# zeyadmohamedabdo/Visual-Question-Answering-VQA-system

Hardware: AMD Instinct MI355X
Metric: image-question pairs/sec (train step) (higher is better)
Workload: dtype bf16

## Files before the change

### visual-question-answering-vqa-system_amd/csrc/cnn_ops.hip

```cpp
#include "common.h"
#include "stem_route.h"

__global__ void bn_reduce_partials_kernel(const float* __restrict__ part, double* __restrict__ acc, int tiles, int C) {
  const int c = blockIdx.x * 64 + (threadIdx.x & 63), tl = threadIdx.x >> 6;
  __shared__ double sh[2][4][64];
  double s = 0.0, q = 0.0;
  if (c < C) {
    const int step = gridDim.y * 4;
    int t = blockIdx.y * 4 + tl;
    for (; t + 7 * step < tiles; t += 8 * step) {
      float a[8], b[8];
#pragma unroll
      for (int u = 0; u < 8; ++u) { a[u] = part[((size_t)(t + u * step) * 2) * C + c]; b[u] = part[((size_t)(t + u * step) * 2 + 1) * C + c]; }
#pragma unroll
      for (int u = 0; u < 8; ++u) { s += (double)a[u]; q += (double)b[u]; }
    }
    for (; t < tiles; t += step) {
      s += (double)part[((size_t)t * 2) * C + c];
      q += (double)part[((size_t)t * 2 + 1) * C + c];
    }
  }
  sh[0][tl][threadIdx.x & 63] = s; sh[1][tl][threadIdx.x & 63] = q;
  __syncthreads();
  if (tl == 0 && c < C) {
// ... 314 lines not shown
    const int ch = c0 + j;
    a[j] = cf[ch]; b[j] = cf[C + ch]; c[j] = cf[2 * C + ch];
    if (DUAL) { a2[j] = cf[3 * C + ch]; b2[j] = cf[4 * C + ch]; c2[j] = cf[5 * C + ch]; }
    if (SELF) { ms[j] = coef[ch]; mh[j] = coef[C + ch]; }
  }
#pragma unroll 2
  for (size_t r = (size_t)blockIdx.x * lanes_r + myr; r < rows; r += (size_t)gridDim.x * lanes_r) {
    const size_t off = r * C + c0;
    Vec16<T> d = ldg16(dout + off), yy = ldg16(y + off), o, y2v, rr, r2;
    if (!SELF && outact) o = ldg16(outact + off);
    if (DUAL) y2v = ldg16(y2 + off);
#pragma unroll
    for (int j = 0; j < VEC; ++j) {
      float g = d.get(j);
      if (SELF) { if (!(yy.get(j) * ms[j] + mh[j] > 0.f)) g = 0.f; }
      else if (outact && !(o.get(j) > 0.f)) g = 0.f;
      rr.set(j, a[j] * g + b[j] * yy.get(j) + c[j]);
      if (DUAL) r2.set(j, a2[j] * g + b2[j] * y2v.get(j) + c2[j]);
    }
    stg16(dy + off, rr);
    if (DUAL) stg16(dy2 + off, r2);
  }
}

constexpr int SP_ROWS = 4, SP_PAIRS = 7;
template <typename T>
__global__ __launch_bounds__(256) void stem_pool_fwd_kernel(const T* __restrict__ y, const float* __restrict__ coef, T* __restrict__ out,
                                                            uint8_t* __restrict__ idx, int B, int H, int W, int C, int Ho, int Wo, int trows) {
  constexpr int VEC = Vec16<T>::N;
  const int cv = C / VEC, Wp = (Wo + 1) >> 1;
  const int tiles_x = (Wp + SP_PAIRS - 1) / SP_PAIRS, tiles_y = (Ho + trows - 1) / trows;
  const int per_row = SP_PAIRS * cv;
  const int ry = threadIdx.x / per_row, rem = threadIdx.x - ry * per_row;
  if (ry >= trows) return;
  const int pr = rem / cv, c0 = (rem - pr * cv) * VEC;
  int t = blockIdx.x;
  const int tx = t % tiles_x; t /= tiles_x; const int ty = t % tiles_y; const int b = t / tiles_y;
  const int oh = ty * trows + ry, owp = tx * SP_PAIRS + pr;
  if (oh >= Ho || owp >= Wp) return;
  float sc[VEC], sh[VEC];
#pragma unroll
  for (int j = 0; j < VEC; ++j) { sc[j] = coef[c0 + j]; sh[j] = coef[C + c0 + j]; }
  const int ow0 = owp * 2;
  const bool two = ow0 + 1 < Wo;
  float best[2][VEC]; int bi[2][VEC];
#pragma unroll
  for (int o = 0; o < 2; ++o)
#pragma unroll
    for (int j = 0; j < VEC; ++j) { best[o][j] = -INFINITY; bi[o][j] = 0; }
#pragma unroll
  for (int r = 0; r < 3; ++r) {
    const int ih = oh * 2 - 1 + r;
    if (ih < 0 || ih >= H) continue;
    const T* yr = y + (((size_t)b * H + ih) * W) * C + c0;
#pragma unroll
    for (int s5 = 0; s5 < 5; ++s5) {
      const int iw = ow0 * 2 - 1 + s5;
      if (iw < 0 || iw >= W) continue;
      const Vec16<T> yy = ldg16(yr + (size_t)iw * C);
      float a[VEC];
#pragma unroll
      for (int j = 0; j < VEC; ++j) { const float v = yy.get(j) * sc[j] + sh[j]; a[j] = v < 0.f ? 0.f : v; }
      if (s5 < 3) {
#pragma unroll
        for (int j = 0; j < VEC; ++j)
          if (a[j] > best[0][j] || a[j] != a[j]) { best[0][j] = a[j]; bi[0][j] = r * 3 + s5; }
      }
      if (s5 >= 2) {
#pragma unroll
        for (int j = 0; j < VEC; ++j)
          if (a[j] > best[1][j] || a[j] != a[j]) { best[1][j] = a[j]; bi[1][j] = r * 3 + s5 - 2; }
      }
    }
  }
#pragma unroll
  for (int o = 0; o < 2; ++o) {
    if (o == 1 && !two) break;
    const size_t e = ((((size_t)b * Ho + oh) * Wo + ow0 + o) * C + c0);
    Vec16<T> ov;
    uint32_t pk[VEC / 4];
#pragma unroll
    for (int q4 = 0; q4 < VEC / 4; ++q4) pk[q4] = 0u;
#pragma unroll
    for (int j = 0; j < VEC; ++j) { ov.set(j, best[o][j]); pk[j >> 2] |= (uint32_t)bi[o][j] << (8 * (j & 3)); }
    stg16(out + e, ov);
#pragma unroll
    for (int q4 = 0; q4 < VEC / 4; ++q4) reinterpret_cast<uint32_t*>(idx + e)[q4] = pk[q4];
  }
}

template <typename T>
__global__ __launch_bounds__(256) void stem_bwd_reduce_kernel(const T* __restrict__ dpool, const uint8_t* __restrict__ idx, const T* __restrict__ y,
                                                              const float* __restrict__ coef, float* __restrict__ slab,
                                                              int B, int H, int W, int C, int Ho, int Wo) {
  constexpr int VEC = Vec16<T>::N;
  const int cv = C / VEC, lanes_r = 256 / cv;
  const int myv = threadIdx.x % cv, myr = threadIdx.x / cv, c0 = myv * VEC;
  const size_t rows = (size_t)B * H * W;
  float sg[VEC], sx[VEC], g[VEC], sc[VEC], sh[VEC], mean[VEC], inv[VEC];
#pragma unroll
  for (int j = 0; j < VEC; ++j) { sg[j] = sx[j] = 0.f; sc[j] = coef[c0 + j]; sh[j] = coef[C + c0 + j]; mean[j] = coef[2 * C + c0 + j]; inv[j] = coef[3 * C + c0 + j]; }
  if (myr < lanes_r)
    for (size_t r = (size_t)blockIdx.x * lanes_r + myr; r < rows; r += (size_t)gridDim.x * lanes_r) {
      const int w = (int)(r % W); size_t q = r / W; const int h = (int)(q % H); const int b = (int)(q / H);
      Vec16<T> yy = ldg16(y + r * C + c0);
      stem_route<T>(dpool, idx, yy, sc, sh, b, h, w, c0, C, Ho, Wo, g);
#pragma unroll
      for (int j = 0; j < VEC; ++j) { sg[j] += g[j]; sx[j] += g[j] * (yy.get(j) - mean[j]) * inv[j]; }
    }
  extern __shared__ float shm[];
#pragma unroll
  for (int j = 0; j < VEC; ++j) { shm[(0 * 256 + threadIdx.x) * VEC + j] = sg[j]; shm[(1 * 256 + threadIdx.x) * VEC + j] = sx[j]; }
  __syncthreads();
  for (int o = threadIdx.x; o < 2 * C; o += 256) {
    const int k = o / C, c = o - k * C, v = c / VEC, j = c - v * VEC;
    float s = 0.f;
    for (int r = 0; r < lanes_r; ++r) s += shm[(k * 256 + r * cv + v) * VEC + j];
    slab[((size_t)blockIdx.x * 3 + k) * C + c] = s;
    if (k == 0) slab[((size_t)blockIdx.x * 3 + 2) * C + c] = 0.f;
  }
}

template <typename T>
__global__ void stem_bwd_apply_kernel(const T* __restrict__ dpool, const uint8_t* __restrict__ idx, const T* __restrict__ y,
                                      const float* __restrict__ coef, const float* __restrict__ bc, T* __restrict__ dy,
                                      int B, int H, int W, int C, int Ho, int Wo) {
  constexpr int VEC = Vec16<T>::N;
  const int cv = C / VEC;
  const size_t total = (size_t)B * H * W * cv;
  float g[VEC];
  for (size_t i = (size_t)blockIdx.x * blockDim.x + threadIdx.x; i < total; i += (size_t)gridDim.x * blockDim.x) {
    const int v = (int)(i % cv); size_t r = i / cv;
    const int w = (int)(r % W); size_t q = r / W; const int h = (int)(q % H); const int b = (int)(q / H);
    const int c0 = v * VEC;
    Vec16<T> yy = ldg16(y + i * VEC), o;
    float sc[VEC], sh[VEC];
#pragma unroll
    for (int j = 0; j < VEC; ++j) { sc[j] = coef[c0 + j]; sh[j] = coef[C + c0 + j]; }
    stem_route<T>(dpool, idx, yy, sc, sh, b, h, w, c0, C, Ho, Wo, g);
#pragma unroll
    for (int j = 0; j < VEC; ++j) o.set(j, bc[c0 + j] * g[j] + bc[C + c0 + j] * yy.get(j) + bc[2 * C + c0 + j]);
    stg16(dy + i * VEC, o);
  }
}

template <typename T>
__global__ __launch_bounds__(256) void se_pool_fc_kernel(const T* __restrict__ x, const float* __restrict__ w1, const float* __restrict__ w2,
                                                         float* __restrict__ pooled, float* __restrict__ hidden, float* __restrict__ scale,
                                                         int HW, int C, int Cr, const float* __restrict__ part, int chunks) {
  constexpr int VEC = Vec16<T>::N;
  extern __shared__ float sh[];
  const int b = blockIdx.x, cv = C / VEC, lanes_r = 256 / cv;
  const int myv = threadIdx.x % cv, myr = threadIdx.x / cv;
  float s[VEC];
#pragma unroll
  for (int j = 0; j < VEC; ++j) s[j] = 0.f;
  if (!part && myr < lanes_r) {
    const T* xb = x + (size_t)b * HW * C + myv * VEC;
    int p = myr;
    for (; p + 3 * lanes_r < HW; p += 4 * lanes_r) {
      Vec16<T> v0 = ldg16(xb + (size_t)p * C), v1 = ldg16(xb + (size_t)(p + lanes_r) * C);
      Vec16<T> v2 = ldg16(xb + (size_t)(p + 2 * lanes_r) * C), v3 = ldg16(xb + (size_t)(p + 3 * lanes_r) * C);
#pragma unroll
      for (int j = 0; j < VEC; ++j) s[j] += (v0.get(j) + v1.get(j)) + (v2.get(j) + v3.get(j));
    }
    for (; p < HW; p += lanes_r) {
      Vec16<T> v = ldg16(xb + (size_t)p * C);
// ... 861 lines not shown
```

### visual-question-answering-vqa-system_amd/csrc/common.h

```cpp
#pragma once
#include <hip/hip_runtime.h>
#include <stdint.h>

#include <stdlib.h>

#ifdef VQA_ABLATION
static inline int vqa_env_int(const char* name, int dflt) { const char* e = getenv(name); return e ? atoi(e) : dflt; }
#else
static inline int vqa_env_int(const char*, int dflt) { return dflt; }
#endif

#define VQA_OK 0
#define VQA_EARG 1000

typedef uint16_t bf16_t;
typedef __attribute__((ext_vector_type(4))) float f32x4;
typedef __attribute__((ext_vector_type(8))) __bf16 bf16x8;
typedef __attribute__((ext_vector_type(4))) short i16x4;
typedef __attribute__((ext_vector_type(4))) uint32_t u32x4;

__device__ __forceinline__ float bf2f(bf16_t v) { return __uint_as_float(((uint32_t)v) << 16); }
__device__ __forceinline__ bf16_t f2bf(float f) {
  __bf16 b = (__bf16)f;
  return __builtin_bit_cast(bf16_t, b);
}
template <typename T> __device__ __forceinline__ float to_f(T v);
template <> __device__ __forceinline__ float to_f<float>(float v) { return v; }
template <> __device__ __forceinline__ float to_f<bf16_t>(bf16_t v) { return bf2f(v); }
template <typename T> __device__ __forceinline__ T from_f(float v);
template <> __device__ __forceinline__ float from_f<float>(float v) { return v; }
template <> __device__ __forceinline__ bf16_t from_f<bf16_t>(float v) { return f2bf(v); }

template <typename T> struct Vec16;
template <> struct Vec16<float> {
  static constexpr int N = 4;
  u32x4 raw;
  __device__ __forceinline__ float get(int i) const { return __uint_as_float(raw[i]); }
  __device__ __forceinline__ void set(int i, float v) { raw[i] = __float_as_uint(v); }
};
template <> struct Vec16<bf16_t> {
  static constexpr int N = 8;
  u32x4 raw;
  __device__ __forceinline__ float get(int i) const {
    uint32_t w = raw[i >> 1];
    return __uint_as_float((i & 1) ? (w & 0xffff0000u) : (w << 16));
  }
  __device__ __forceinline__ void set(int i, float v) {
    uint32_t b = f2bf(v);
    uint32_t w = raw[i >> 1];
    raw[i >> 1] = (i & 1) ? ((w & 0x0000ffffu) | (b << 16)) : ((w & 0xffff0000u) | b);
  }
};
template <typename T> __device__ __forceinline__ Vec16<T> ldg16(const T* p) {
  Vec16<T> v; v.raw = *reinterpret_cast<const u32x4*>(p); return v;
}
template <typename T> __device__ __forceinline__ void stg16(T* p, const Vec16<T>& v) {
  *reinterpret_cast<u32x4*>(p) = v.raw;
}
template <typename T> __device__ __forceinline__ Vec16<T> zero16() {
  Vec16<T> v; v.raw = u32x4{0u, 0u, 0u, 0u}; return v;
}

__device__ __forceinline__ float wave_sum(float v) {
#pragma unroll
  for (int o = 32; o > 0; o >>= 1) v += __shfl_xor(v, o, 64);
  return v;
}
__device__ __forceinline__ float wave_max(float v) {
#pragma unroll
  for (int o = 32; o > 0; o >>= 1) v = fmaxf(v, __shfl_xor(v, o, 64));
  return v;
}

__device__ __forceinline__ uint32_t mix32(uint32_t x) {
  x ^= x >> 16; x *= 0x7feb352dU; x ^= x >> 15; x *= 0x846ca68bU; x ^= x >> 16; return x;
}
__device__ __forceinline__ uint32_t drop_key(uint64_t seed) { return mix32((uint32_t)seed) ^ (uint32_t)(seed >> 32) * 0x9E3779B9u; }
__device__ __forceinline__ bool drop_keep32(uint32_t key, uint32_t idx, float p) {
  const uint32_t h = mix32(idx ^ key);
  return (float)(h >> 8) * (1.0f / 16777216.0f) >= p;
}
__device__ __forceinline__ bool drop_keep(uint64_t seed, uint64_t idx, float p) {
  uint32_t h = mix32((uint32_t)idx ^ mix32((uint32_t)(idx >> 32) + (uint32_t)seed) ^ (uint32_t)(seed >> 32) * 0x9E3779B9u);
  return (float)(h >> 8) * (1.0f / 16777216.0f) >= p;
}

static inline __host__ __device__ int acc_replicas(int C) { const int r = 512 / (C > 0 ? C : 1); return r < 1 ? 1 : (r > 8 ? 8 : r); }
#define VQA_ACC_HI_SHIFT 4
#define VQA_ACC_LO_SHIFT 50
#define VQA_ACC_MAX_PARTS (1 << 17)
#define VQA_ACC_LIMIT_LOG2 (62 - VQA_ACC_HI_SHIFT - 17)
__device__ __forceinline__ void acc_add_fixed(unsigned long long* acc, size_t n, size_t idx, float v) {
  constexpr float lim = (float)(1ull << VQA_ACC_LIMIT_LOG2), hs = (float)(1 << VQA_ACC_HI_SHIFT), lscale = (float)(1ull << VQA_ACC_LO_SHIFT);
  if (fabsf(v) < lim) {
    const float hi = rintf(v * hs);
    const float lo = __builtin_fmaf(hi, -1.f / hs, v);
    atomicAdd(acc + idx, (unsigned long long)(long long)hi);
    if (lo != 0.f) atomicAdd(acc + n + 1 + idx, (unsigned long long)__float2ll_rn(lo * lscale));
  } else atomicAdd(acc + n, 1ull);
}
__device__ __forceinline__ double acc_read_fixed(const unsigned long long* acc, int R, int K, int C, int k, int c) {
  const size_t n = (size_t)R * K * C;
  long long h[8], l[8];
#pragma unroll
  for (int r = 0; r < 8; ++r) {
    const size_t i = ((size_t)r * K + k) * C + c;
    h[r] = r < R ? (long long)acc[i] : 0ll;
// ... 33 lines not shown
```

### visual-question-answering-vqa-system_amd/csrc/stem_conv.hip

```cpp
#include <cstdlib>
#include "common.h"
#include <type_traits>
#include "stem_route.h"

namespace {
constexpr int RB = 4;
constexpr int PR = 2 * RB + 5;
constexpr int KP = 192;
constexpr int LDW = KP + 8;
constexpr int LDCS = 64 + 8;
}

template <int PROWS, int XO, int CH>
__device__ __forceinline__ void stem_fill_patch(bf16_t* __restrict__ patch, int PW, __amdgpu_buffer_rsrc_t rsImg, int b, int ih_base,
                                                int H, int W, int tid) {
  static_assert(XO & 1, "odd column offset");
  const int W4 = W >> 2, nitems = 3 * PROWS * W4, nh = PW - W;
  const float inv_w4 = 1.0f / (float)W4, inv_nh = 1.0f / (float)nh;
  for (int i = tid; i < 3 * PROWS * nh; i += 256) {
    const int row = (int)(((float)i + 0.5f) * inv_nh), k = i - row * nh;
    patch[row * PW + (k < XO ? k : W + k)] = 0;
  }
  for (int base = tid; base < nitems; base += 256 * CH) {
    f32x4 v[CH]; int dst[CH];
#pragma unroll
    for (int i = 0; i < CH; ++i) {
      const int id = base + 256 * i;
      dst[i] = -1;
      v[i] = f32x4{0.f, 0.f, 0.f, 0.f};
      if (id < nitems) {
        const int row = (int)(((float)id + 0.5f) * inv_w4), j = id - row * W4;
        const int c = row / PROWS, pr = row - c * PROWS, ih = ih_base + pr;
        dst[i] = row * PW + 4 * j + XO;
        if (ih >= 0 && ih < H)
          v[i] = __builtin_bit_cast(f32x4, __builtin_amdgcn_raw_buffer_load_b128(rsImg, (((b * 3 + c) * H + ih) * W + 4 * j) * 4, 0, 0));
      }
    }
#pragma unroll
    for (int i = 0; i < CH; ++i) {
      if (dst[i] < 0) continue;
      bf16_t* d = patch + dst[i];
      d[0] = f2bf(v[i][0]);
      *reinterpret_cast<uint32_t*>(d + 1) = (uint32_t)f2bf(v[i][1]) | ((uint32_t)f2bf(v[i][2]) << 16);
      d[3] = f2bf(v[i][3]);
    }
  }
}

__global__ void stem_pack_kernel(const float* __restrict__ w, bf16_t* __restrict__ out) {
  const int i = blockIdx.x * blockDim.x + threadIdx.x;
  if (i >= 64 * KP) return;
  const int n = i / KP, k = i - n * KP, pair = k >> 3, s = k & 7;
  float v = 0.f;
  if (pair < 21 && s < 7) { const int c = pair / 7, r = pair - c * 7; v = w[((n * 7 + r) * 7 + s) * 3 + c]; }
  out[i] = f2bf(v);
}

__global__ __launch_bounds__(256) void stem_conv_kernel(const float* __restrict__ img, const bf16_t* __restrict__ wst, bf16_t* __restrict__ out,
                                                        float* __restrict__ stats, int H, int W, int Ho, int Wo) {
  extern __shared__ __attribute__((aligned(16))) char smem[];
  const int PW = 2 * Wo + 8;
  bf16_t* patch = reinterpret_cast<bf16_t*>(smem);
  bf16_t* Wl = patch + 3 * PR * PW;
  bf16_t* Cst = Wl;
  float* red = reinterpret_cast<float*>(Wl + 64 * LDW);
  const int tid = threadIdx.x, lane = tid & 63, wave = tid >> 6, g = lane >> 4, li = lane & 15;
  const int rblocks = Ho / RB;
  const int b = blockIdx.x / rblocks, oh0 = (blockIdx.x - b * rblocks) * RB;

  for (int v = tid; v < 64 * (KP / 8); v += 256) {
    const int n = v / (KP / 8), kv = v - n * (KP / 8);
    *reinterpret_cast<u32x4*>(&Wl[n * LDW + kv * 8]) = *reinterpret_cast<const u32x4*>(&wst[n * KP + kv * 8]);
  }
  const int ih_base = 2 * oh0 - 3;
  const __amdgpu_buffer_rsrc_t rsImg = __builtin_amdgcn_make_buffer_rsrc(const_cast<float*>(img), 0, (int)gridDim.x / rblocks * 3 * H * W * 4, 0x00020000);
  for (int x = tid; x < PW; x += 256) {
    const int iw = x - 3;
    const bool cok = iw >= 0 && iw < W;
    float vals[3 * PR];
#pragma unroll
    for (int row = 0; row < 3 * PR; ++row) {
      const int c = row / PR, pr = row - c * PR, ih = ih_base + pr;
// ... 122 lines not shown
  for (int kk = 0; kk < 6; ++kk)
#pragma unroll
    for (int nt = 0; nt < 4; ++nt)
      bfr[kk][nt] = *reinterpret_cast<const bf16x8*>(&Wl[(nt * 16 + li) * LDW + kk * 32 + g * 8]);
  float sc[4], sh[4];
#pragma unroll
  for (int nt = 0; nt < 4; ++nt) { sc[nt] = coef[nt * 16 + li]; sh[nt] = coef[64 + nt * 16 + li]; }
  __syncthreads();
  if (dbg & 4) { if (tid == 0) out[(size_t)blockIdx.x * 64] = f2bf(sc[0] + (float)bfr[0][0][0]); return; }

  bf16_t* mycs = Cst + wave * 8 * LDCS;
  for (int t = wave; t < ctiles; t += 4) {
    const int c0 = 14 * t - 1;
    auto row = [&](int i, float (&h)[4][2]) {
      f32x4 acc[4];
#pragma unroll
      for (int nt = 0; nt < 4; ++nt) acc[nt] = f32x4{0.f, 0.f, 0.f, 0.f};
      if (!(dbg & 1))
#pragma unroll
      for (int kk = 0; kk < 6; ++kk) {
        int pair = kk * 4 + g;
        pair = pair > 20 ? 20 : pair;
        const int c = pair / 7, r = pair - c * 7;
        const uint32_t* ap = reinterpret_cast<const uint32_t*>(&patch[(c * PRP + 2 * i + r) * PW + 28 * t + 2 * li]);
        u32x4 raw = {ap[0], ap[1], ap[2], ap[3]};
        const bf16x8 af = __builtin_bit_cast(bf16x8, raw);
#pragma unroll
        for (int nt = 0; nt < 4; ++nt) acc[nt] = __builtin_amdgcn_mfma_f32_16x16x32_bf16(af, bfr[kk][nt], acc[nt], 0, 0, 0);
      }
      if (dbg & 2) {
#pragma unroll
        for (int nt = 0; nt < 4; ++nt) { h[nt][0] = acc[nt][0] + acc[nt][1]; h[nt][1] = acc[nt][2] + acc[nt][3]; }
        return;
      }
#pragma unroll
      for (int nt = 0; nt < 4; ++nt) {
        float v[4];
#pragma unroll
        for (int r4 = 0; r4 < 4; ++r4) {
          const int col = c0 + 4 * g + r4;
          const float a = acc[nt][r4] * sc[nt] + sh[nt];
          v[r4] = ((unsigned)col < (unsigned)Wo) ? (a < 0.f ? 0.f : a) : 0.f;
        }
        const float nx = __shfl_down(v[0], 16, 64);
        h[nt][0] = pool_max(pool_max(v[0], v[1]), v[2]);
        h[nt][1] = pool_max(pool_max(v[2], v[3]), nx);
      }
    };
    float hp[4][2], h1[4][2], h2[4][2];
    if (ph0 > 0) row(0, hp);
    else {
#pragma unroll
      for (int nt = 0; nt < 4; ++nt) { hp[nt][0] = 0.f; hp[nt][1] = 0.f; }
    }
#pragma unroll 1
    for (int k = 0; k < PRB; ++k) {
      row(2 * k + 1, h1);
      row(2 * k + 2, h2);
#pragma unroll
      for (int nt = 0; nt < 4; ++nt)
#pragma unroll
        for (int q = 0; q < 2; ++q) {
          const float o = pool_max(pool_max(hp[nt][q], h1[nt][q]), h2[nt][q]);
          mycs[(2 * g + q) * LDCS + nt * 16 + li] = f2bf(o);
          hp[nt][q] = h2[nt][q];
        }
      asm volatile("s_waitcnt lgkmcnt(0)" ::: "memory");
      const int px = lane >> 3, cv = lane & 7, pw = 7 * t + px;
      if (px < 7 && pw < Wp)
        *reinterpret_cast<u32x4*>(&out[((((size_t)b * Hp + ph0 + k) * Wp + pw) * 64) + cv * 8]) = *reinterpret_cast<const u32x4*>(&mycs[px * LDCS + cv * 8]);
      asm volatile("s_waitcnt lgkmcnt(0)" ::: "memory");
    }
  }
}

namespace {
constexpr int RBW = 4;
constexpr int PRW = 2 * RBW + 5;
constexpr int LDA = KP + 8;
constexpr int LDD = 64 + 4;
}

template <bool FUSED>
__global__ __launch_bounds__(256) void stem_wgrad_kernel(const float* __restrict__ img, const bf16_t* __restrict__ dy, float* __restrict__ dw,
                                                         int B, int H, int W, int Ho, int Wo, const bf16_t* __restrict__ dpool,
                                                         const uint8_t* __restrict__ idx, const float* __restrict__ coef,
                                                         const float* __restrict__ bc, int Hp, int Wp, int nsplit, float* __restrict__ ws) {
  extern __shared__ __attribute__((aligned(16))) char smem[];
  const int PW = 2 * Wo + 8;
  const int Wh = Wo / nsplit;
  const int MP = (Wh + 31) / 32 * 32;
  bf16_t* patch = reinterpret_cast<bf16_t*>(smem);
  bf16_t* Acol = patch + 3 * PRW * PW;
  bf16_t* Dy = Acol + MP * LDA;
  const int tid = threadIdx.x, lane = tid & 63, wave = tid >> 6, g = lane >> 4, li = lane & 15;
  const int q = li >> 2, pp = li & 3;
  for (int i = tid; i < (MP - Wh) * LDA; i += 256) Acol[Wh * LDA + i] = 0;
  for (int i = tid; i < (MP - Wh) * LDD; i += 256) Dy[Wh * LDD + i] = 0;

  float f_sc[8], f_sh[8], f_a[8], f_b[8], f_c[8];
  if (FUSED) {
    const int c0f = (tid & 7) * 8;
#pragma unroll
    for (int j = 0; j < 8; ++j) {
      f_sc[j] = coef[c0f + j]; f_sh[j] = coef[64 + c0f + j];
      f_a[j] = bc[c0f + j]; f_b[j] = bc[64 + c0f + j]; f_c[j] = bc[128 + c0f + j];
    }
  }
  const __amdgpu_buffer_rsrc_t rsP = __builtin_amdgcn_make_buffer_rsrc(const_cast<bf16_t*>(FUSED ? dpool : dy), 0, FUSED ? B * Hp * Wp * 64 * 2 : 0, 0x00020000);
  const __amdgpu_buffer_rsrc_t rsI = __builtin_amdgcn_make_buffer_rsrc(const_cast<uint8_t*>(FUSED ? idx : reinterpret_cast<const uint8_t*>(dy)), 0, FUSED ? B * Hp * Wp * 64 : 0, 0x00020000);
  const __amdgpu_buffer_rsrc_t rsImg = __builtin_amdgcn_make_buffer_rsrc(const_cast<float*>(img), 0, B * 3 * H * W * 4, 0x00020000);
  const __amdgpu_buffer_rsrc_t rsDy = __builtin_amdgcn_make_buffer_rsrc(const_cast<bf16_t*>(dy), 0, B * Ho * Wo * 64 * 2, 0x00020000);
  f32x4 acc[4][3];
#pragma unroll
  for (int i = 0; i < 4; ++i)
#pragma unroll
    for (int j = 0; j < 3; ++j) acc[i][j] = f32x4{0.f, 0.f, 0.f, 0.f};

  const int rblocks = Ho / RBW, nblocks = B * rblocks;
  for (int blk = blockIdx.x; blk < nblocks; blk += gridDim.x) {
    const int b = blk / rblocks, oh0 = (blk - b * rblocks) * RBW;
    __syncthreads();
    const int ih_base = 2 * oh0 - 3;
    for (int x = tid; x < PW; x += 256) {
      const int iw = x - 3;
      const bool cok = iw >= 0 && iw < W;
      float vals[3 * PRW];
#pragma unroll
      for (int row = 0; row < 3 * PRW; ++row) {
        const int c = row / PRW, pr = row - c * PRW, ih = ih_base + pr;
        const bool ok = cok && ih >= 0 && ih < H;
        const int ihc = min(max(ih, 0), H - 1), iwc = min(max(iw, 0), W - 1);
        const float t = __builtin_bit_cast(float, __builtin_amdgcn_raw_buffer_load_b32(rsImg, (((b * 3 + c) * H + ihc) * W + iwc) * 4, 0, 0));
        vals[row] = ok ? t : 0.f;
      }
#pragma unroll
      for (int row = 0; row < 3 * PRW; ++row) patch[row * PW + x] = f2bf(vals[row]);
    }
    for (int unit = 0; unit < RBW * nsplit; ++unit) {
      const int orow = unit / nsplit, px0 = (unit - orow * nsplit) * Wh;
      __syncthreads();
      const int dyr_b = (((b * Ho + oh0 + orow) * Wo + px0) * 64) * 2;
      if constexpr (FUSED) {
        auto stage_row = [&](auto odd) {
          for (int v = tid; v < (Wh >> 1) * 8; v += 256) {
            const int pq = v >> 3, cv = v & 7;
            Vec16<bf16_t> yy[2];
            yy[0].raw = __builtin_bit_cast(u32x4, __builtin_amdgcn_raw_buffer_load_b128(rsDy, dyr_b + (2 * pq) * 128 + cv * 16, 0, 0));
            yy[1].raw = __builtin_bit_cast(u32x4, __builtin_amdgcn_raw_buffer_load_b128(rsDy, dyr_b + (2 * pq + 1) * 128 + cv * 16, 0, 0));
            float g8[2][8];
            stem_route_pair_buf<decltype(odd)::value>(rsP, rsI, yy, f_sc, f_sh, b, oh0 + orow, (px0 >> 1) + pq, cv * 8, Hp, Wp, g8);
#pragma unroll
            for (int q2 = 0; q2 < 2; ++q2) {
              Vec16<bf16_t> o;
#pragma unroll
              for (int j = 0; j < 8; ++j) o.set(j, f_a[j] * g8[q2][j] + f_b[j] * yy[q2].get(j) + f_c[j]);
              uint32_t* d = reinterpret_cast<uint32_t*>(&Dy[(2 * pq + q2) * LDD + cv * 8]);
              d[0] = o.raw[0]; d[1] = o.raw[1]; d[2] = o.raw[2]; d[3] = o.raw[3];
            }
          }
        };
        if ((oh0 + orow) & 1) stage_row(std::true_type{});
        else stage_row(std::false_type{});
      } else {
        for (int v = tid; v < Wh * 8; v += 256) {
          const int px = v >> 3, cv = v & 7;
          const u32x4 val = __builtin_bit_cast(u32x4, __builtin_amdgcn_raw_buffer_load_b128(rsDy, dyr_b + v * 16, 0, 0));
          uint32_t* d = reinterpret_cast<uint32_t*>(&Dy[px * LDD + cv * 8]);
          d[0] = val[0]; d[1] = val[1]; d[2] = val[2]; d[3] = val[3];
        }
      }
      if (tid < 240) {
        const int pair = tid % 24, c = pair / 7, r = pair - c * 7;
        const bf16_t* prow = patch + (c * PRW + 2 * orow + r) * PW + 2 * px0;
        for (int px = tid / 24; px < Wh; px += 10) {
          u32x4 val = {0u, 0u, 0u, 0u};
          if (pair < 21) {
            const uint32_t* ap = reinterpret_cast<const uint32_t*>(prow + 2 * px);
            val = u32x4{ap[0], ap[1], ap[2], ap[3] & 0x0000ffffu};
          }
          *reinterpret_cast<u32x4*>(&Acol[px * LDA + pair * 8]) = val;
        }
      }
      __syncthreads();
      typedef __attribute__((ext_vector_type(8))) short i16x8;
      for (int ks = 0; ks < MP / 32; ++ks) {
        const bf16_t* yb = Dy + (ks * 32 + 8 * g + q) * LDD + 4 * pp;
        const bf16_t* xb = Acol + (ks * 32 + 8 * g + q) * LDA + wave * 48 + 4 * pp;
        bf16x8 af[4], bfv[3];
#pragma unroll
        for (int i = 0; i < 4; ++i) {
          i16x4 lo = __builtin_amdgcn_ds_read_tr16_b64_v4i16((i16x4 __attribute__((address_space(3)))*)(yb + i * 16));
          i16x4 hi = __builtin_amdgcn_ds_read_tr16_b64_v4i16((i16x4 __attribute__((address_space(3)))*)(yb + 4 * LDD + i * 16));
          i16x8 t = {lo[0], lo[1], lo[2], lo[3], hi[0], hi[1], hi[2], hi[3]};
          af[i] = __builtin_bit_cast(bf16x8, t);
        }
#pragma unroll
        for (int j = 0; j < 3; ++j) {
          i16x4 lo = __builtin_amdgcn_ds_read_tr16_b64_v4i16((i16x4 __attribute__((address_space(3)))*)(xb + j * 16));
          i16x4 hi = __builtin_amdgcn_ds_read_tr16_b64_v4i16((i16x4 __attribute__((address_space(3)))*)(xb + 4 * LDA + j * 16));
          i16x8 t = {lo[0], lo[1], lo[2], lo[3], hi[0], hi[1], hi[2], hi[3]};
          bfv[j] = __builtin_bit_cast(bf16x8, t);
        }
#pragma unroll
        for (int i = 0; i < 4; ++i)
#pragma unroll
          for (int j = 0; j < 3; ++j)
            acc[i][j] = __builtin_amdgcn_mfma_f32_16x16x32_bf16(af[i], bfv[j], acc[i][j], 0, 0, 0);
      }
    }
  }
#pragma unroll
  for (int j = 0; j < 3; ++j) {
    const int k2 = wave * 48 + j * 16 + li, pair = k2 >> 3, s = k2 & 7;
    if (pair >= 21 || s >= 7) continue;
    const int c = pair / 7, r = pair - c * 7;
#pragma unroll
    for (int i = 0; i < 4; ++i)
#pragma unroll
      for (int rr = 0; rr < 4; ++rr) {
        const size_t o = (size_t)(i * 16 + g * 4 + rr) * 147 + (r * 7 + s) * 3 + c;
        if (ws) ws[(size_t)blockIdx.x * (64 * 147) + o] = acc[i][j][rr];
        else atomicAdd(dw + o, acc[i][j][rr]);
      }
  }
}

extern "C" int vqa_slab_reduce(const float* ws, float* dw, int nslabs, long long n, hipStream_t st);

static size_t stem_wgrad_shm(int Wo, int nsplit) {
  const int PW = 2 * Wo + 8, MP = (Wo / nsplit + 31) / 32 * 32;
  return (size_t)(3 * PRW * PW + MP * LDA + MP * LDD) * 2;
}
static int stem_nsplit(int Wo) {
  const int env = vqa_env_int("VQA_STEM_NSPLIT", 0);
  if (env > 0 && Wo % (8 * env) == 0) return env;
  const int floor_ = Wo > 64 ? 2 : 1;
  for (int n = floor_; n <= 16; ++n)
    if (Wo % (8 * n) == 0 && stem_wgrad_shm(Wo, n) <= (size_t)160 * 1024 / 3) return n;
  return floor_;
}
static int stem_wgrad_grid(int B, int Ho, int Wo, size_t* shm_out) {
  const size_t shm = stem_wgrad_shm(Wo, stem_nsplit(Wo));
  if (shm_out) *shm_out = shm;
  if (shm > 160 * 1024) return 0;
  const int nblocks = B * (Ho / RBW);
  const int cap = 256 * (int)((160 * 1024) / shm > 4 ? 4 : (160 * 1024) / shm);
  return nblocks < cap ? nblocks : cap;
}

extern "C" {

int vqa_stem_conv_blocks(int B, int H, int W) {
  const int Ho = (H + 6 - 7) / 2 + 1, Wo = (W + 6 - 7) / 2 + 1;
  if (Ho % RB || Wo % 16 || Wo > 256) return 0;
  return B * (Ho / RB);
}
int vqa_stem_pack(const float* w_krsc, void* wstem , hipStream_t st) {
  if (!w_krsc || !wstem) return VQA_EARG;
  hipLaunchKernelGGL(stem_pack_kernel, dim3((64 * KP + 255) / 256), dim3(256), 0, st, w_krsc, (bf16_t*)wstem);
  VQA_LAUNCH_CHECK(); return VQA_OK;
}
int vqa_stem_conv(const float* img, const void* wstem, void* out, float* stats, int B, int H, int W, hipStream_t st) {
  const int nb = vqa_stem_conv_blocks(B, H, W);
  if (!img || !wstem || !out || nb <= 0 || (size_t)B * 3 * H * W * 4 >= 0x7fffffffull) return VQA_EARG;
  const int Ho = (H + 6 - 7) / 2 + 1, Wo = (W + 6 - 7) / 2 + 1, PW = 2 * Wo + 8;
  const size_t shm = (size_t)(3 * PR * PW + 64 * LDW) * 2 + 4 * 64 * 2 * 4;
  static size_t attr = 0;
  if (shm > attr) { (void)hipFuncSetAttribute(reinterpret_cast<const void*>(&stem_conv_kernel), hipFuncAttributeMaxDynamicSharedMemorySize, (int)shm); attr = shm; }
  hipLaunchKernelGGL(stem_conv_kernel, dim3(nb), dim3(256), shm, st, img, (const bf16_t*)wstem, (bf16_t*)out, stats, H, W, Ho, Wo);
  VQA_LAUNCH_CHECK(); return VQA_OK;
}

static size_t stem_conv_pool_shm(int H, int W, int* ctiles_out, int* pw_out) {
  const int Ho = (H + 6 - 7) / 2 + 1, Wo = (W + 6 - 7) / 2 + 1, Hp = (Ho + 2 - 3) / 2 + 1, Wp = (Wo + 2 - 3) / 2 + 1;
  if (H < 7 || W < 7 || (Ho & 1) || (Wo & 1) || Hp % PRB) return 0;
  const int ctiles = (Wp + 6) / 7;
  const int PW = (2 * (14 * ctiles + 2) + 8 + 7) / 8 * 8;
  if (ctiles_out) *ctiles_out = ctiles;
  if (pw_out) *pw_out = PW;
  const size_t shm = (size_t)(3 * PRP * PW + 64 * LDW) * 2;
  return shm <= 160 * 1024 ? shm : 0;
}
int vqa_stem_conv_pool_ok(int B, int H, int W) {
  return B > 0 && stem_conv_pool_shm(H, W, nullptr, nullptr) > 0 && (size_t)B * 3 * H * W * 4 < 0x7fffffffull;
}
int vqa_stem_conv_pool(const float* img, const void* wstem, const float* coef, void* out, int B, int H, int W, hipStream_t st) {
  int ctiles = 0, PW = 0;
  const size_t shm = stem_conv_pool_shm(H, W, &ctiles, &PW);
  if (!img || !wstem || !coef || !out || !vqa_stem_conv_pool_ok(B, H, W)) return VQA_EARG;
  const int Ho = (H + 6 - 7) / 2 + 1, Wo = (W + 6 - 7) / 2 + 1, Hp = (Ho + 2 - 3) / 2 + 1, Wp = (Wo + 2 - 3) / 2 + 1;
  static size_t attr = 0;
  if (shm > attr) { (void)hipFuncSetAttribute(reinterpret_cast<const void*>(&stem_conv_pool_kernel), hipFuncAttributeMaxDynamicSharedMemorySize, (int)shm); attr = shm; }
  hipLaunchKernelGGL(stem_conv_pool_kernel, dim3(B * (Hp / PRB)), dim3(256), shm, st, img, (const bf16_t*)wstem, coef, (bf16_t*)out,
                     B, H, W, Ho, Wo, Hp, Wp, ctiles, PW, vqa_env_int("VQA_STEMCP_DBG", 0));
  VQA_LAUNCH_CHECK(); return VQA_OK;
}

int vqa_stem_wgrad_blocks(int B, int H, int W) {
  const int Ho = (H + 6 - 7) / 2 + 1, Wo = (W + 6 - 7) / 2 + 1;
  if (Ho % RBW || Wo % 16 || Wo > 256) return 0;
  return stem_wgrad_grid(B, Ho, Wo, nullptr);
}

int vqa_stem_wgrad(const float* img, const void* dy, float* dw, int B, int H, int W, float* ws, long long ws_floats, hipStream_t st) {
  const int Ho = (H + 6 - 7) / 2 + 1, Wo = (W + 6 - 7) / 2 + 1;
  if (!img || !dy || !dw || Ho % RBW || Wo % 16 || Wo > 256) return VQA_EARG;
  if ((size_t)B * Ho * Wo * 64 * 2 >= 0x7fffffffull || (size_t)B * 3 * H * W * 4 >= 0x7fffffffull) return VQA_EARG;
  const int nsplit = stem_nsplit(Wo);
  const int PW = 2 * Wo + 8, MP = (Wo / nsplit + 31) / 32 * 32;
  const size_t shm = (size_t)(3 * PRW * PW + MP * LDA + MP * LDD) * 2;
  if (shm > 160 * 1024) return VQA_EARG;
  static size_t attr = 0;
  if (shm > attr) { (void)hipFuncSetAttribute(reinterpret_cast<const void*>(&stem_wgrad_kernel<false>), hipFuncAttributeMaxDynamicSharedMemorySize, (int)shm); attr = shm; }
  int nblocks = B * (Ho / RBW);
  const int cap = 256 * (int)((160 * 1024) / shm > 4 ? 4 : (160 * 1024) / shm);
  int grid = nblocks < cap ? nblocks : cap;
  float* w = (ws && ws_floats >= (long long)grid * 64 * 147) ? ws : nullptr;
  hipLaunchKernelGGL(stem_wgrad_kernel<false>, dim3(grid), dim3(256), shm, st, img, (const bf16_t*)dy, dw, B, H, W, Ho, Wo,
                     (const bf16_t*)nullptr, (const uint8_t*)nullptr, (const float*)nullptr, (const float*)nullptr, 0, 0, nsplit, w);
  VQA_LAUNCH_CHECK();
  return w ? vqa_slab_reduce(w, dw, grid, 64 * 147, st) : VQA_OK;
}
int vqa_stem_wgrad_fused(const float* img, const void* y, const void* dpool, const uint8_t* idx, const float* coef, const float* bcoef,
                         float* dw, int B, int H, int W, float* ws, long long ws_floats, hipStream_t st) {
  const int Ho = (H + 6 - 7) / 2 + 1, Wo = (W + 6 - 7) / 2 + 1, Hp = (Ho + 2 - 3) / 2 + 1, Wp = (Wo + 2 - 3) / 2 + 1;
  if (!img || !y || !dpool || !idx || !coef || !bcoef || !dw || Ho % RBW || Wo % 16 || Wo > 256) return VQA_EARG;
  if ((size_t)B * Ho * Wo * 64 * 2 >= 0x7fffffffull || (size_t)B * 3 * H * W * 4 >= 0x7fffffffull) return VQA_EARG;
  const int nsplit = stem_nsplit(Wo);
  const int PW = 2 * Wo + 8, MP = (Wo / nsplit + 31) / 32 * 32;
  const size_t shm = (size_t)(3 * PRW * PW + MP * LDA + MP * LDD) * 2;
  if (shm > 160 * 1024) return VQA_EARG;
  static size_t attr = 0;
  if (shm > attr) { (void)hipFuncSetAttribute(reinterpret_cast<const void*>(&stem_wgrad_kernel<true>), hipFuncAttributeMaxDynamicSharedMemorySize, (int)shm); attr = shm; }
  int nblocks = B * (Ho / RBW);
  const int cap = 256 * (int)((160 * 1024) / shm > 4 ? 4 : (160 * 1024) / shm);
  int grid = nblocks < cap ? nblocks : cap;
  float* w = (ws && ws_floats >= (long long)grid * 64 * 147) ? ws : nullptr;
  hipLaunchKernelGGL(stem_wgrad_kernel<true>, dim3(grid), dim3(256), shm, st, img, (const bf16_t*)y, dw, B, H, W, Ho, Wo,
                     (const bf16_t*)dpool, idx, coef, bcoef, Hp, Wp, nsplit, w);
  VQA_LAUNCH_CHECK();
  return w ? vqa_slab_reduce(w, dw, grid, 64 * 147, st) : VQA_OK;
}

}
```

### visual-question-answering-vqa-system_amd/csrc/stem_route.h

```cpp
#pragma once
#include "common.h"

template <typename T>
__device__ __forceinline__ void stem_route(const T* __restrict__ dpool, const uint8_t* __restrict__ idx, const Vec16<T>& yy,
                                           const float* sc, const float* sh, int b, int h, int w, int c0, int C, int Ho, int Wo, float* g) {
  constexpr int VEC = Vec16<T>::N;
#pragma unroll
  for (int j = 0; j < VEC; ++j) g[j] = 0.f;
  const int oh_a = (h - 1) >> 1, oh_b = (h + 1) >> 1, ow_a = (w - 1) >> 1, ow_b = (w + 1) >> 1;
  Vec16<T> d[4]; uint64_t iw4[4]; bool ok[4]; int code[4];
#pragma unroll
  for (int k = 0; k < 4; ++k) {
    const int oh = (k >> 1) ? oh_b : oh_a, ow = (k & 1) ? ow_b : ow_a;
    const int r = h - (oh * 2 - 1), s = w - (ow * 2 - 1);
    ok[k] = oh >= 0 && oh < Ho && ow >= 0 && ow < Wo && r >= 0 && r <= 2 && s >= 0 && s <= 2 &&
            !((k >> 1) && oh_b == oh_a) && !((k & 1) && ow_b == ow_a);
    code[k] = r * 3 + s;
    const int ohc = min(max(oh, 0), Ho - 1), owc = min(max(ow, 0), Wo - 1);
    const size_t o = (((size_t)b * Ho + ohc) * Wo + owc) * C + c0;
    d[k] = ldg16(dpool + o);
    if constexpr (VEC == 8) iw4[k] = *reinterpret_cast<const uint64_t*>(idx + o);
    else iw4[k] = *reinterpret_cast<const uint32_t*>(idx + o);
  }
#pragma unroll
  for (int k = 0; k < 4; ++k)
#pragma unroll
    for (int j = 0; j < VEC; ++j) {
      const int id = (int)((iw4[k] >> (8 * j)) & 0xff);
      if (ok[k] && id == code[k]) g[j] += d[k].get(j);
    }
#pragma unroll
  for (int j = 0; j < VEC; ++j)
    if (!(yy.get(j) * sc[j] + sh[j] > 0.f)) g[j] = 0.f;
}

__device__ __forceinline__ void stem_route_buf(__amdgpu_buffer_rsrc_t rsP, __amdgpu_buffer_rsrc_t rsI, const Vec16<bf16_t>& yy,
                                               const float* sc, const float* sh, int b, int h, int w, int c0, int Ho, int Wo, float* g) {
#pragma unroll
  for (int j = 0; j < 8; ++j) g[j] = 0.f;
  const int oh_a = (h - 1) >> 1, oh_b = (h + 1) >> 1, ow_a = (w - 1) >> 1, ow_b = (w + 1) >> 1;
  Vec16<bf16_t> d[4]; uint32_t ilo[4], ihi[4]; int code[4];
#pragma unroll
  for (int k = 0; k < 4; ++k) {
    const int oh = (k >> 1) ? oh_b : oh_a, ow = (k & 1) ? ow_b : ow_a;
    const int r = h - (oh * 2 - 1), s = w - (ow * 2 - 1);
    const bool ok = oh >= 0 && oh < Ho && ow >= 0 && ow < Wo && r >= 0 && r <= 2 && s >= 0 && s <= 2 &&
                    !((k >> 1) && oh_b == oh_a) && !((k & 1) && ow_b == ow_a);
    code[k] = ok ? r * 3 + s : 255;
    const int ohc = min(max(oh, 0), Ho - 1), owc = min(max(ow, 0), Wo - 1);
    const int o = ((b * Ho + ohc) * Wo + owc) * 64 + c0;
    d[k].raw = __builtin_bit_cast(u32x4, __builtin_amdgcn_raw_buffer_load_b128(rsP, o * 2, 0, 0));
    typedef __attribute__((ext_vector_type(2))) unsigned u32x2_t;
    const u32x2_t iw = __builtin_bit_cast(u32x2_t, __builtin_amdgcn_raw_buffer_load_b64(rsI, o, 0, 0));
    ilo[k] = iw[0]; ihi[k] = iw[1];
  }
#pragma unroll
  for (int k = 0; k < 4; ++k)
#pragma unroll
    for (int j = 0; j < 8; ++j) {
      const int id = (int)(((j < 4 ? ilo[k] : ihi[k]) >> (8 * (j & 3))) & 0xff);
      if (id == code[k]) g[j] += d[k].get(j);
    }
#pragma unroll
  for (int j = 0; j < 8; ++j)
    if (!(yy.get(j) * sc[j] + sh[j] > 0.f)) g[j] = 0.f;
}

template <bool ODD>
__device__ __forceinline__ void stem_route_pair_buf(__amdgpu_buffer_rsrc_t rsP, __amdgpu_buffer_rsrc_t rsI, const Vec16<bf16_t> (&yy)[2],
                                                    const float* sc, const float* sh, int b, int h, int j, int c0, int Ho, int Wo,
                                                    float (&g)[2][8]) {
  typedef __attribute__((ext_vector_type(2))) unsigned u32x2_t;
#pragma unroll
  for (int q = 0; q < 2; ++q)
#pragma unroll
    for (int jx = 0; jx < 8; ++jx) g[q][jx] = 0.f;
  constexpr int NP = ODD ? 2 : 1;
#pragma unroll
  for (int kr = 0; kr < NP; ++kr) {
    const int oh = ODD ? ((h - 1) >> 1) + kr : (h >> 1);
    const int r = ODD ? (kr ? 0 : 2) : 1;
    const bool rok = oh >= 0 && oh < Ho;
    const int ohc = min(max(oh, 0), Ho - 1);
    Vec16<bf16_t> d[2]; u32x2_t iw[2]; bool ok[2];
#pragma unroll
    for (int kc = 0; kc < 2; ++kc) {
      const int ow = j + kc;
      ok[kc] = rok && ow < Wo;
      const int o = ((b * Ho + ohc) * Wo + min(ow, Wo - 1)) * 64 + c0;
      d[kc].raw = __builtin_bit_cast(u32x4, __builtin_amdgcn_raw_buffer_load_b128(rsP, o * 2, 0, 0));
      iw[kc] = __builtin_bit_cast(u32x2_t, __builtin_amdgcn_raw_buffer_load_b64(rsI, o, 0, 0));
    }
    const int c_e = ok[0] ? r * 3 + 1 : 255, c_o0 = ok[0] ? r * 3 + 2 : 255, c_o1 = ok[1] ? r * 3 : 255;
#pragma unroll
    for (int jx = 0; jx < 8; ++jx) {
      const int i0 = (int)((iw[0][jx >> 2] >> (8 * (jx & 3))) & 0xff), i1 = (int)((iw[1][jx >> 2] >> (8 * (jx & 3))) & 0xff);
      const float d0 = d[0].get(jx), d1 = d[1].get(jx);
      if (i0 == c_e) g[0][jx] += d0;
      if (i0 == c_o0) g[1][jx] += d0;
      if (i1 == c_o1) g[1][jx] += d1;
    }
  }
#pragma unroll
  for (int q = 0; q < 2; ++q)
#pragma unroll
    for (int jx = 0; jx < 8; ++jx)
      if (!(yy[q].get(jx) * sc[jx] + sh[jx] > 0.f)) g[q][jx] = 0.f;
}
```

Baseline: 43130.

## Encode ReLU mask into pool indices and streamline stem wgrad staging

The maxpool forward now writes a masked marker into the argmax index whenever the pooled value is non-positive. The fused stem weight-gradient kernel can therefore drop its per-element BN/ReLU recompute and the coefficient registers it needed. The wgrad kernel also gains launch bounds for 3 blocks per SIMD, packed bf16 conversion, and an im2col staging loop that writes two rows per iteration from overlapping loads. The shared-memory attribute is now set once per device through an atomic bitmask. The risk is that the mask equivalence (pooled max > 0 versus per-pixel BN output > 0) must hold exactly, and the new register cap may cause spills.

```diff
diff --git a/visual-question-answering-vqa-system_amd/csrc/cnn_ops.hip b/visual-question-answering-vqa-system_amd/csrc/cnn_ops.hip
--- a/visual-question-answering-vqa-system_amd/csrc/cnn_ops.hip
+++ b/visual-question-answering-vqa-system_amd/csrc/cnn_ops.hip
@@ -420,7 +420,10 @@
 #pragma unroll
     for (int q4 = 0; q4 < VEC / 4; ++q4) pk[q4] = 0u;
 #pragma unroll
-    for (int j = 0; j < VEC; ++j) { ov.set(j, best[o][j]); pk[j >> 2] |= (uint32_t)bi[o][j] << (8 * (j & 3)); }
+    for (int j = 0; j < VEC; ++j) {
+      ov.set(j, best[o][j]);
+      pk[j >> 2] |= (uint32_t)(best[o][j] > 0.f ? bi[o][j] : STEM_IDX_MASKED) << (8 * (j & 3));
+    }
     stg16(out + e, ov);
 #pragma unroll
     for (int q4 = 0; q4 < VEC / 4; ++q4) reinterpret_cast<uint32_t*>(idx + e)[q4] = pk[q4];
diff --git a/visual-question-answering-vqa-system_amd/csrc/common.h b/visual-question-answering-vqa-system_amd/csrc/common.h
--- a/visual-question-answering-vqa-system_amd/csrc/common.h
+++ b/visual-question-answering-vqa-system_amd/csrc/common.h
@@ -23,6 +23,11 @@
 __device__ __forceinline__ bf16_t f2bf(float f) {
   __bf16 b = (__bf16)f;
   return __builtin_bit_cast(bf16_t, b);
+}
+__device__ __forceinline__ uint32_t f2bf_pk(float lo, float hi) {
+  typedef __attribute__((ext_vector_type(2))) float f32x2_t;
+  typedef __attribute__((ext_vector_type(2))) __bf16 bf16x2_t;
+  return __builtin_bit_cast(uint32_t, __builtin_convertvector((f32x2_t){lo, hi}, bf16x2_t));
 }
 template <typename T> __device__ __forceinline__ float to_f(T v);
 template <> __device__ __forceinline__ float to_f<float>(float v) { return v; }
diff --git a/visual-question-answering-vqa-system_amd/csrc/stem_conv.hip b/visual-question-answering-vqa-system_amd/csrc/stem_conv.hip
--- a/visual-question-answering-vqa-system_amd/csrc/stem_conv.hip
+++ b/visual-question-answering-vqa-system_amd/csrc/stem_conv.hip
@@ -1,3 +1,4 @@
+#include <atomic>
 #include <cstdlib>
 #include "common.h"
 #include <type_traits>
@@ -286,7 +287,7 @@
 }
 
 template <bool FUSED>
-__global__ __launch_bounds__(256) void stem_wgrad_kernel(const float* __restrict__ img, const bf16_t* __restrict__ dy, float* __restrict__ dw,
+__global__ __launch_bounds__(256, 3) void stem_wgrad_kernel(const float* __restrict__ img, const bf16_t* __restrict__ dy, float* __restrict__ dw,
                                                          int B, int H, int W, int Ho, int Wo, const bf16_t* __restrict__ dpool,
                                                          const uint8_t* __restrict__ idx, const float* __restrict__ coef,
                                                          const float* __restrict__ bc, int Hp, int Wp, int nsplit, float* __restrict__ ws) {
@@ -301,15 +302,13 @@
   const int q = li >> 2, pp = li & 3;
   for (int i = tid; i < (MP - Wh) * LDA; i += 256) Acol[Wh * LDA + i] = 0;
   for (int i = tid; i < (MP - Wh) * LDD; i += 256) Dy[Wh * LDD + i] = 0;
-
-  float f_sc[8], f_sh[8], f_a[8], f_b[8], f_c[8];
+  for (int i = tid; i < Wh * 24; i += 256) Acol[(i / 24) * LDA + 168 + (i % 24)] = 0;
+
+  float f_a[8], f_b[8], f_c[8];
   if (FUSED) {
     const int c0f = (tid & 7) * 8;
 #pragma unroll
-    for (int j = 0; j < 8; ++j) {
-      f_sc[j] = coef[c0f + j]; f_sh[j] = coef[64 + c0f + j];
-      f_a[j] = bc[c0f + j]; f_b[j] = bc[64 + c0f + j]; f_c[j] = bc[128 + c0f + j];
-    }
+    for (int j = 0; j < 8; ++j) { f_a[j] = bc[c0f + j]; f_b[j] = bc[64 + c0f + j]; f_c[j] = bc[128 + c0f + j]; }
   }
   const __amdgpu_buffer_rsrc_t rsP = __builtin_amdgcn_make_buffer_rsrc(const_cast<bf16_t*>(FUSED ? dpool : dy), 0, FUSED ? B * Hp * Wp * 64 * 2 : 0, 0x00020000);
   const __amdgpu_buffer_rsrc_t rsI = __builtin_amdgcn_make_buffer_rsrc(const_cast<uint8_t*>(FUSED ? idx : reinterpret_cast<const uint8_t*>(dy)), 0, FUSED ? B * Hp * Wp * 64 : 0, 0x00020000);
@@ -353,14 +352,15 @@
             yy[0].raw = __builtin_bit_cast(u32x4, __builtin_amdgcn_raw_buffer_load_b128(rsDy, dyr_b + (2 * pq) * 128 + cv * 16, 0, 0));
             yy[1].raw = __builtin_bit_cast(u32x4, __builtin_amdgcn_raw_buffer_load_b128(rsDy, dyr_b + (2 * pq + 1) * 128 + cv * 16, 0, 0));
             float g8[2][8];
-            stem_route_pair_buf<decltype(odd)::value>(rsP, rsI, yy, f_sc, f_sh, b, oh0 + orow, (px0 >> 1) + pq, cv * 8, Hp, Wp, g8);
+            stem_route_pair_buf<decltype(odd)::value>(rsP, rsI, b, oh0 + orow, (px0 >> 1) + pq, cv * 8, Hp, Wp, g8);
 #pragma unroll
             for (int q2 = 0; q2 < 2; ++q2) {
-              Vec16<bf16_t> o;
-#pragma unroll
-              for (int j = 0; j < 8; ++j) o.set(j, f_a[j] * g8[q2][j] + f_b[j] * yy[q2].get(j) + f_c[j]);
+              float o[8];
+#pragma unroll
+              for (int j = 0; j < 8; ++j) o[j] = f_a[j] * g8[q2][j] + f_b[j] * yy[q2].get(j) + f_c[j];
               uint32_t* d = reinterpret_cast<uint32_t*>(&Dy[(2 * pq + q2) * LDD + cv * 8]);
-              d[0] = o.raw[0]; d[1] = o.raw[1]; d[2] = o.raw[2]; d[3] = o.raw[3];
+#pragma unroll
+              for (int k = 0; k < 4; ++k) d[k] = f2bf_pk(o[2 * k], o[2 * k + 1]);
             }
           }
         };
@@ -374,16 +374,16 @@
           d[0] = val[0]; d[1] = val[1]; d[2] = val[2]; d[3] = val[3];
         }
       }
-      if (tid < 240) {
-        const int pair = tid % 24, c = pair / 7, r = pair - c * 7;
+      if (const int t2 = (tid - (Wh >> 1) * 8) & 255; t2 < 252) {
+        typedef __attribute__((ext_vector_type(2))) unsigned u32x2_t;
+        const int pair = t2 % 21, c = pair / 7, r = pair - c * 7;
         const bf16_t* prow = patch + (c * PRW + 2 * orow + r) * PW + 2 * px0;
-        for (int px = tid / 24; px < Wh; px += 10) {
-          u32x4 val = {0u, 0u, 0u, 0u};
-          if (pair < 21) {
-            const uint32_t* ap = reinterpret_cast<const uint32_t*>(prow + 2 * px);
-            val = u32x4{ap[0], ap[1], ap[2], ap[3] & 0x0000ffffu};
-          }
-          *reinterpret_cast<u32x4*>(&Acol[px * LDA + pair * 8]) = val;
+        for (int m = t2 / 21; m < (Wh >> 1); m += 12) {
+          const bf16_t* ap = prow + 4 * m;
+          const u32x2_t w01 = *reinterpret_cast<const u32x2_t*>(ap), w23 = *reinterpret_cast<const u32x2_t*>(ap + 4);
+          const uint32_t w4 = *reinterpret_cast<const uint32_t*>(ap + 8);
+          *reinterpret_cast<u32x4*>(&Acol[(2 * m) * LDA + pair * 8]) = u32x4{w01[0], w01[1], w23[0], w23[1]};
+          *reinterpret_cast<u32x4*>(&Acol[(2 * m + 1) * LDA + pair * 8]) = u32x4{w01[1], w23[0], w23[1], w4};
         }
       }
       __syncthreads();
@@ -431,6 +431,15 @@
 }
 
 extern "C" int vqa_slab_reduce(const float* ws, float* dw, int nslabs, long long n, hipStream_t st);
+
+static void stem_allow_lds(const void* kern, std::atomic<uint64_t>& done) {
+  int dev = 0;
+  if (hipGetDevice(&dev) != hipSuccess) dev = 0;
+  const uint64_t bit = dev >= 0 && dev < 64 ? 1ull << dev : 0ull;
+  if (bit && (done.load(std::memory_order_acquire) & bit)) return;
+  (void)hipFuncSetAttribute(kern, hipFuncAttributeMaxDynamicSharedMemorySize, 160 * 1024);
+  if (bit) done.fetch_or(bit, std::memory_order_release);
+}
 
 static size_t stem_wgrad_shm(int Wo, int nsplit) {
   const int PW = 2 * Wo + 8, MP = (Wo / nsplit + 31) / 32 * 32;
@@ -515,8 +524,8 @@
   const int PW = 2 * Wo + 8, MP = (Wo / nsplit + 31) / 32 * 32;
   const size_t shm = (size_t)(3 * PRW * PW + MP * LDA + MP * LDD) * 2;
   if (shm > 160 * 1024) return VQA_EARG;
-  static size_t attr = 0;
-  if (shm > attr) { (void)hipFuncSetAttribute(reinterpret_cast<const void*>(&stem_wgrad_kernel<false>), hipFuncAttributeMaxDynamicSharedMemorySize, (int)shm); attr = shm; }
+  static std::atomic<uint64_t> lds_set{0};
+  stem_allow_lds(reinterpret_cast<const void*>(&stem_wgrad_kernel<false>), lds_set);
   int nblocks = B * (Ho / RBW);
   const int cap = 256 * (int)((160 * 1024) / shm > 4 ? 4 : (160 * 1024) / shm);
   int grid = nblocks < cap ? nblocks : cap;
@@ -535,8 +544,8 @@
   const int PW = 2 * Wo + 8, MP = (Wo / nsplit + 31) / 32 * 32;
   const size_t shm = (size_t)(3 * PRW * PW + MP * LDA + MP * LDD) * 2;
   if (shm > 160 * 1024) return VQA_EARG;
-  static size_t attr = 0;
-  if (shm > attr) { (void)hipFuncSetAttribute(reinterpret_cast<const void*>(&stem_wgrad_kernel<true>), hipFuncAttributeMaxDynamicSharedMemorySize, (int)shm); attr = shm; }
+  static std::atomic<uint64_t> lds_set{0};
+  stem_allow_lds(reinterpret_cast<const void*>(&stem_wgrad_kernel<true>), lds_set);
   int nblocks = B * (Ho / RBW);
   const int cap = 256 * (int)((160 * 1024) / shm > 4 ? 4 : (160 * 1024) / shm);
   int grid = nblocks < cap ? nblocks : cap;
diff --git a/visual-question-answering-vqa-system_amd/csrc/stem_route.h b/visual-question-answering-vqa-system_amd/csrc/stem_route.h
--- a/visual-question-answering-vqa-system_amd/csrc/stem_route.h
+++ b/visual-question-answering-vqa-system_amd/csrc/stem_route.h
@@ -1,5 +1,9 @@
 #pragma once
 #include "common.h"
+
+constexpr int STEM_IDX_MASKED = 254;
+constexpr int STEM_CODE_NONE = 255;
+static_assert(STEM_IDX_MASKED > 8 && STEM_IDX_MASKED != STEM_CODE_NONE && STEM_IDX_MASKED < 256, "marker: no position code, no sentinel");
 
 template <typename T>
 __device__ __forceinline__ void stem_route(const T* __restrict__ dpool, const uint8_t* __restrict__ idx, const Vec16<T>& yy,
@@ -46,7 +50,7 @@
     const int r = h - (oh * 2 - 1), s = w - (ow * 2 - 1);
     const bool ok = oh >= 0 && oh < Ho && ow >= 0 && ow < Wo && r >= 0 && r <= 2 && s >= 0 && s <= 2 &&
                     !((k >> 1) && oh_b == oh_a) && !((k & 1) && ow_b == ow_a);
-    code[k] = ok ? r * 3 + s : 255;
+    code[k] = ok ? r * 3 + s : STEM_CODE_NONE;
     const int ohc = min(max(oh, 0), Ho - 1), owc = min(max(ow, 0), Wo - 1);
     const int o = ((b * Ho + ohc) * Wo + owc) * 64 + c0;
     d[k].raw = __builtin_bit_cast(u32x4, __builtin_amdgcn_raw_buffer_load_b128(rsP, o * 2, 0, 0));
@@ -67,9 +71,8 @@
 }
 
 template <bool ODD>
-__device__ __forceinline__ void stem_route_pair_buf(__amdgpu_buffer_rsrc_t rsP, __amdgpu_buffer_rsrc_t rsI, const Vec16<bf16_t> (&yy)[2],
-                                                    const float* sc, const float* sh, int b, int h, int j, int c0, int Ho, int Wo,
-                                                    float (&g)[2][8]) {
+__device__ __forceinline__ void stem_route_pair_buf(__amdgpu_buffer_rsrc_t rsP, __amdgpu_buffer_rsrc_t rsI, int b, int h, int j, int c0,
+                                                    int Ho, int Wo, float (&g)[2][8]) {
   typedef __attribute__((ext_vector_type(2))) unsigned u32x2_t;
 #pragma unroll
   for (int q = 0; q < 2; ++q)
@@ -91,19 +94,14 @@
       d[kc].raw = __builtin_bit_cast(u32x4, __builtin_amdgcn_raw_buffer_load_b128(rsP, o * 2, 0, 0));
       iw[kc] = __builtin_bit_cast(u32x2_t, __builtin_amdgcn_raw_buffer_load_b64(rsI, o, 0, 0));
     }
-    const int c_e = ok[0] ? r * 3 + 1 : 255, c_o0 = ok[0] ? r * 3 + 2 : 255, c_o1 = ok[1] ? r * 3 : 255;
+    const int c_e = ok[0] ? r * 3 + 1 : STEM_CODE_NONE, c_o0 = ok[0] ? r * 3 + 2 : STEM_CODE_NONE, c_o1 = ok[1] ? r * 3 : STEM_CODE_NONE;
 #pragma unroll
     for (int jx = 0; jx < 8; ++jx) {
       const int i0 = (int)((iw[0][jx >> 2] >> (8 * (jx & 3))) & 0xff), i1 = (int)((iw[1][jx >> 2] >> (8 * (jx & 3))) & 0xff);
       const float d0 = d[0].get(jx), d1 = d[1].get(jx);
-      if (i0 == c_e) g[0][jx] += d0;
-      if (i0 == c_o0) g[1][jx] += d0;
-      if (i1 == c_o1) g[1][jx] += d1;
+      g[0][jx] += i0 == c_e ? d0 : 0.f;
+      g[1][jx] += i0 == c_o0 ? d0 : 0.f;
+      g[1][jx] += i1 == c_o1 ? d1 : 0.f;
     }
   }
-#pragma unroll
-  for (int q = 0; q < 2; ++q)
-#pragma unroll
-    for (int jx = 0; jx < 8; ++jx)
-      if (!(yy[q].get(jx) * sc[jx] + sh[jx] > 0.f)) g[q][jx] = 0.f;
 }
```

Result: no change. 43500, median of 6 (+0.9%).
